# jarek1992/raytracer_project

Measured on AMD Instinct MI355X. Metric: Msamples/sec (rays·bounces), higher is better.
Workload: dtype f64

## Files before the change

### include/zr_capi.h

```cpp
#ifndef ZR_CAPI_H
#define ZR_CAPI_H

#include <stddef.h>
#include <stdint.h>

#ifdef __cplusplus
extern "C" {
#endif

#define ZR_ABI_VERSION 3

enum {
    ZR_OK = 0,
    ZR_E_INVALID = -1,
    ZR_E_DEVICE = -2,
    ZR_E_STATE = -3,
    ZR_E_CANCELLED = -4,
    ZR_E_NOMEM = -5
};

enum {
    ZR_PRIM_SPHERE = 0,
    ZR_PRIM_TRIANGLE = 1,
    ZR_PRIM_CUBE = 2,
// ... 358 lines not shown
    uint32_t leaf;
    uint32_t kind;
    uint32_t count;
    uint32_t first;
    uint32_t subtree;
    uint32_t src[4];
} zr_tree_box;
int zr_scene_tree_boxes(const zr_scene*, zr_tree_box* out, size_t cap);

#define ZR_PATH_RECORD 17
int zr_trace_paths(zr_ctx*, const zr_scene*, const zr_camera*, uint64_t seed, const int32_t* requests, int n, int max_segments, double* out);

int zr_get_counters(zr_ctx*, zr_counters*);
uint64_t zr_last_presolved_pixels(zr_ctx*);
int zr_last_round_loop(zr_ctx*, int* drain_round, int* sub_pools);
int zr_get_kernel_times(zr_ctx*, float* ms, int cap);

#define ZR_COMM_ID_BYTES 128
typedef struct zr_comm zr_comm;
int zr_comm_unique_id(unsigned char id[ZR_COMM_ID_BYTES]);
zr_comm* zr_comm_create(zr_ctx*, int nranks, int rank, const unsigned char id[ZR_COMM_ID_BYTES]);
int zr_comm_reduce_frame(zr_comm*, void* d_frame, size_t n_doubles, int root, void* hip_stream);
int zr_comm_gather_frame(zr_comm*, void* d_frame, int W, int H, const zr_region* region, int root, void* hip_stream);
void zr_comm_destroy(zr_comm*);

int zr_trace(zr_ctx*, const zr_scene*, const double* rays6, size_t n, double tmin, double tmax,
             uint64_t seed, uint64_t pixel, uint32_t bounce, zr_hit* out);

typedef struct zr_scatter_out {
    double attenuation[3], origin[3], direction[3];
// ... 17 lines not shown
```

### raytracer_project_amd/capi.py

```python
import ctypes as C
import os

import numpy as np

_HERE = os.path.dirname(os.path.abspath(__file__))
LIB_PATH = os.environ.get("ZR_LIB") or os.path.join(_HERE, "csrc", "libzr_hip.so")
SCENES_LIB_PATH = os.path.join(_HERE, "csrc", "libzr_scenes.so")

ZR_OK, ZR_E_INVALID, ZR_E_DEVICE, ZR_E_STATE, ZR_E_CANCELLED, ZR_E_NOMEM = 0, -1, -2, -3, -4, -5
NO_TEXTURE = 0xFFFFFFFF


class XformOp(C.Structure):
    _fields_ = [("kind", C.c_uint32), ("mat", C.c_uint32), ("a", C.c_double * 3)]


class Object(C.Structure):
    _fields_ = [("type", C.c_uint32), ("index", C.c_uint32), ("chain_first", C.c_uint32), ("chain_count", C.c_uint32)]


class Medium(C.Structure):
    _fields_ = [("boundary_type", C.c_uint32), ("boundary_index", C.c_uint32), ("chain_first", C.c_uint32),
                ("chain_count", C.c_uint32), ("mat", C.c_uint32), ("pad_", C.c_uint32), ("neg_inv_density", C.c_double)]

# ... 191 lines not shown
_lib = None
_scenes = None

CAPI_SYMBOLS = [
    "zr_abi_version", "zr_last_error", "zr_create", "zr_destroy", "zr_scene_create", "zr_scene_destroy",
    "zr_scene_set_spheres", "zr_scene_set_triangles", "zr_scene_set_triangle_uvs", "zr_scene_set_cubes", "zr_scene_set_media",
    "zr_scene_set_xform_ops", "zr_scene_set_objects", "zr_scene_set_groups", "zr_scene_set_materials", "zr_scene_set_textures",
    "zr_scene_set_all", "zr_scene_set_all_borrowed", "zr_scene_commit", "zr_scene_update_xform_ops", "zr_scene_update_spheres", "zr_scene_refit", "zr_scene_stats", "zr_scene_kernels", "zr_scene_traversal_stack", "zr_scene_builder", "zr_render", "zr_render_device",
    "zr_accum_create", "zr_accum_destroy", "zr_accum_reset", "zr_render_accumulate", "zr_accum_resolve", "zr_accum_resolve_device", "zr_accum_state",
    "zr_render_adaptive", "zr_accum_error", "zr_accum_sample_counts", "zr_accum_lane_sums",
    "zr_render_aov", "zr_render_passes", "zr_trace_paths", "zr_post_process", "zr_analyze_frame", "zr_denoise", "zr_sharpen_frame",
    "zr_accum_variance", "zr_denoise_guided", "zr_accum_denoise",
    "zr_accum_halves", "zr_denoise_nlm", "zr_accum_denoise_nlm",
    "zr_render_gbuffer", "zr_temporal_create", "zr_temporal_destroy", "zr_temporal_reset", "zr_temporal_state", "zr_temporal_accumulate", "zr_accum_temporal",
    "zr_temporal_view",
    "zr_render_bvh_debug", "zr_trace_bvh_debug", "zr_scene_tree_boxes", "zr_get_counters", "zr_last_presolved_pixels", "zr_last_round_loop",
    "zr_get_kernel_times", "zr_trace", "zr_kat_scatter", "zr_kat_shade_lean", "zr_kat_texture", "zr_kat_background", "zr_kat_camera_rays", "zr_comm_unique_id", "zr_comm_create", "zr_comm_reduce_frame", "zr_comm_gather_frame", "zr_comm_destroy",
]


def load():
    global _lib
    if _lib is not None:
        return _lib
    if not os.path.exists(LIB_PATH):
        raise OSError(f"{LIB_PATH} not built: run `python -c 'import __graft_entry__ as g; g.build()'` "
                      "(hipcc --offload-arch=gfx950); there is no CPU fallback")
    lib = C.CDLL(LIB_PATH, mode=C.RTLD_GLOBAL)
    vp, u64, i32 = C.c_void_p, C.c_uint64, C.c_int
    lib.zr_abi_version.restype = i32
    lib.zr_last_error.restype = C.c_char_p
# ... 54 lines not shown
        lib.zr_temporal_reset.argtypes = [vp]
        lib.zr_temporal_state.argtypes = [vp, C.POINTER(C.c_int64 * 4)]
        lib.zr_temporal_accumulate.argtypes = [vp, C.POINTER(TemporalParams), vp, C.POINTER(Camera), u64, vp, vp, vp, vp, vp]
        lib.zr_accum_temporal.argtypes = [vp, vp, C.POINTER(TemporalParams), vp, C.POINTER(Camera), u64, vp, vp, vp]
        lib.zr_temporal_view.argtypes = [C.POINTER(Camera), C.POINTER(C.c_double * 16)]
    lib.zr_render_bvh_debug.argtypes = [vp, vp, C.POINTER(Camera), C.POINTER(Env), u64, C.POINTER(Region), C.POINTER(BvhDebugParams), vp, vp, vp]
    lib.zr_trace_bvh_debug.argtypes = [vp, vp, C.POINTER(BvhDebugParams), vp, C.c_size_t, C.c_double, u64, u64, C.c_uint32, vp]
    lib.zr_scene_tree_boxes.argtypes = [vp, vp, C.c_size_t]
    lib.zr_trace_paths.argtypes = [vp, vp, C.POINTER(Camera), u64, vp, i32, i32, vp]
    lib.zr_render_passes.argtypes = [vp, vp, C.POINTER(Camera), C.POINTER(Env), u64, C.POINTER(Region), vp, vp, vp]
    lib.zr_get_counters.argtypes = [vp, C.POINTER(Counters)]
    if hasattr(lib, "zr_last_presolved_pixels"):
        lib.zr_last_presolved_pixels.argtypes = [vp]; lib.zr_last_presolved_pixels.restype = u64
    if hasattr(lib, "zr_last_round_loop"):
        lib.zr_last_round_loop.argtypes = [vp, C.POINTER(C.c_int), C.POINTER(C.c_int)]
    lib.zr_get_kernel_times.argtypes = [vp, C.POINTER(C.c_float), i32]
    lib.zr_trace.argtypes = [vp, vp, vp, C.c_size_t, C.c_double, C.c_double, u64, u64, C.c_uint32, vp]
    lib.zr_kat_scatter.argtypes = [vp, vp, vp, vp, vp, vp, C.c_size_t, vp]
    if hasattr(lib, "zr_kat_shade_lean"):
        lib.zr_kat_shade_lean.argtypes = [vp, vp, vp, vp, vp, C.c_size_t, vp, vp]
    lib.zr_kat_texture.argtypes = [vp, vp, C.c_uint32, vp, C.c_size_t, vp]
    lib.zr_kat_background.argtypes = [vp, vp, C.POINTER(Env), vp, C.c_size_t, vp]
    lib.zr_kat_camera_rays.argtypes = [vp, C.POINTER(Camera), u64, vp, C.c_size_t, vp]
    lib.zr_comm_unique_id.argtypes = [vp]
    lib.zr_comm_create.restype = vp; lib.zr_comm_create.argtypes = [vp, i32, i32, vp]
    lib.zr_comm_reduce_frame.argtypes = [vp, vp, C.c_size_t, i32, vp]
    lib.zr_comm_gather_frame.argtypes = [vp, vp, i32, i32, C.POINTER(Region), i32, vp]
    lib.zr_comm_destroy.argtypes = [vp]
    _lib = lib
    return lib
# ... 258 lines not shown
        return out

    def counters(self):
        c = Counters()
        _check(self.lib.zr_get_counters(self._c, C.byref(c)))
        return c

    def presolved_pixels(self):
        return int(self.lib.zr_last_presolved_pixels(self._c))

    def round_loop(self):
        d, k = C.c_int(0), C.c_int(0)
        _check(self.lib.zr_last_round_loop(self._c, C.byref(d), C.byref(k)))
        return d.value, k.value

    def kernel_times_ms(self, cap=256):
        buf = (C.c_float * cap)()
        n = self.lib.zr_get_kernel_times(self._c, buf, cap)
        if n < 0:
            _check(n)
        return [buf[i] for i in range(min(n, cap))]


class Accumulator:

    def __init__(self, ctx, width, height, region=None):
        self.ctx = ctx
        self.lib = ctx.lib
        self.width, self.height = int(width), int(height)
        self._a = self.lib.zr_accum_create(ctx._c, self.width, self.height, C.byref(region) if region is not None else None)
# ... 317 lines not shown
```

### raytracer_project_amd/csrc/zr_host_internal.h

```cpp
#pragma once
#include <hip/hip_runtime_api.h>

#include "zr_build.h"
#include "zr_scene_input.h"
#include "zr_launch.h"

#define HIP_OK(expr)                                                                                         \
    do {                                                                                                     \
        hipError_t e_ = (expr);                                                                              \
        if (e_ != hipSuccess) return fail(ZR_E_DEVICE, "%s failed: %s", #expr, hipGetErrorString(e_));       \
    } while (0)

namespace zr_host {

const double kPi = 3.14159265358979323846;

struct H3 { double x, y, z; };
inline H3 h3(const double* p) { return H3{p[0], p[1], p[2]}; }
inline H3 operator+(H3 a, H3 b) { return H3{a.x + b.x, a.y + b.y, a.z + b.z}; }
inline H3 operator-(H3 a, H3 b) { return H3{a.x - b.x, a.y - b.y, a.z - b.z}; }
inline H3 operator-(H3 a) { return H3{-a.x, -a.y, -a.z}; }
inline H3 operator*(double t, H3 v) { return H3{t * v.x, t * v.y, t * v.z}; }
inline H3 operator*(H3 v, double t) { return t * v; }
inline H3 operator/(H3 v, double t) { return (1 / t) * v; }
// ... 55 lines not shown
    DevBuf<uint32_t> d_kend;
    DevBuf<unsigned char> d_cls;
    DevBuf<unsigned long long> d_cpart;
    DevBuf<unsigned int> d_ctl;
    DevBuf<unsigned char> d_st_overflow;
    uint32_t st_ovf_levels = 0;
    int st_blocks = 0;
    int fused_blocks = 0;
    uint32_t st_slots = 0;
    int st_pools = -1;
    hipEvent_t st_event = nullptr;
    unsigned int* h_active = nullptr;
    unsigned int* h_polls = nullptr;
    hipEvent_t poll_events[zr::POLL_RING * ST_MAX_POOLS] = {};
    int last_drain_round = 0, last_sub_pools = 0;
    std::vector<int32_t> pix_key;
    uint64_t last_rounds = 0;
    int last_path = 0;
    double last_extend_ms = 0, last_shade_ms = 0;
    struct Pending { hipEvent_t a, b; uint64_t render_id; int kind; };
    std::vector<hipEvent_t> pool;
    std::vector<Pending> pending;
    std::vector<float> log;
    int log_kind = 1;
    uint64_t render_id = 0;
    double last_render_ms = 0;
    hipStream_t last_stream = nullptr;
    bool last_counted = false;
    std::mutex trash_m;
    std::thread trash;
// ... 58 lines not shown
```

### raytracer_project_amd/csrc/zr_launch.h

```cpp
#pragma once
#include <hip/hip_runtime.h>
#include <stdint.h>
#include "../../include/zr_capi.h"
#include "zr_round_polls.h"

#define ZR_BLOCK 256

namespace zr {

struct DScene;
struct DCamera;
struct DEnv;

enum { CTR_SAMPLES = 0, CTR_SEGMENTS = 1, CTR_NODES = 2, CTR_SPHERES = 3, CTR_TRIANGLES = 4, CTR_CUBES = 5, CTR_MEDIA = 6, CTR_HITS = 7, CTR_DRAWS = 8,
       CTR_NODE_EXECS = 9, CTR_NODE_LANES = 10, CTR_LEAF_EXECS = 11, CTR_LEAF_LANES = 12,
       CTR_SHADE_EXECS = 13, CTR_SHADE_LANES = 14,
       CTR_ESCAPED = 15,
       CTR_WORDS = 16,
       CTR_HIST = 16, CTR_HIST_WORDS = 24,
       CTR_BLOCK = 48 };
enum { CTR_PROF_EXECS = 1, CTR_PROF_LANES = 2,
       CTR_PROF_WAVE_TICKS = 13,
       CTR_PROF_WAVES = 14 };

// ... 38 lines not shown
};
struct StreamPool {
    void* slots; uint32_t P; void* drain; uint32_t drain_slots, unit_chunk;
};
struct StreamContext {
    unsigned int* ctl; void* overflow; uint32_t ovf_levels; int extend_blocks; unsigned long long* gctr;
    hipStream_t* streams; int n_pools;
    hipEvent_t event; unsigned int* h_active;
    unsigned int* h_polls = nullptr; hipEvent_t* poll_events = nullptr;
};
struct StreamSplit { int mode; void* kend; void* cls; unsigned long long* cpart; };
struct StreamHooks {
    StreamTimer* timer; volatile const uint8_t* keep_going ; StreamProgress* progress;
    int* done_out;
    int* drain_out = nullptr;
};
struct StreamJob { StreamFrame frame; StreamPool pool; StreamContext ctx; StreamSplit split; StreamHooks hooks; };
hipError_t stream_render(const DScene& sc, const StreamJob& job, int leaf_level);
#define ZR_FUSED_OBJECTS 16
struct FusedObjs {
    uint32_t n, pad_;
    uint32_t kind[ZR_FUSED_OBJECTS];
    uint32_t index[ZR_FUSED_OBJECTS];
    double rec[ZR_FUSED_OBJECTS][16];
};
int fused_blocks();
hipError_t fused_render_frame(const DScene& sc, const StreamFrame& frame, const StreamContext& ctx, int blocks, int level, const FusedObjs& objs, const StreamHooks& hooks);
constexpr size_t ACCUM_DOUBLES_PER_PIXEL = 192;
hipError_t launch_accumulate(const double* samples, uint32_t n_pix, uint32_t n, uint32_t sample0, bool flip, double* partial, hipStream_t stream);
hipError_t launch_accum_resolve(const double* partial, const uint32_t* pixels, uint32_t n_pix, int W, int done, int asc_lanes, double* out, hipStream_t stream);
// ... 59 lines not shown
```

### raytracer_project_amd/csrc/zr_render.cpp

```cpp
#include "zr_frame.h"

namespace zr_host {
namespace {

size_t batch_tiles(bool interactive) { return (size_t)std::max(1, (int)env_double("ZR_BATCH_TILES", interactive ? 256 : (double)(1 << 30))); }

void make_camera(const zr_camera& c, zr::DCamera& d) {
    int W = c.image_width < 1 ? 1 : c.image_width, H = c.image_height < 1 ? 1 : c.image_height;
    double aspect = double(W) / H;
    H3 center = h3(c.lookfrom), lookat = h3(c.lookat), vup = h3(c.vup);
    double theta = c.vfov * kPi / 180.0;
    double h = std::tan(theta / 2);
    double vh = 2 * h * c.focus_dist;
    double vw = vh * aspect;
    H3 w = unit(center - lookat);
    H3 u = unit(cross(vup, w));
    H3 v = cross(w, u);
    H3 vu = vw * u;
    H3 vv = vh * -v;
    H3 du = vu / W;
    H3 dv = vv / H;
    H3 ul = center - (c.focus_dist * w) - vu / 2 - vv / 2;
    H3 p00 = ul + 0.5 * (du + dv);
    double rad = c.focus_dist * std::tan((c.defocus_angle / 2) * kPi / 180.0);
// ... 342 lines not shown
        for (int y = r.ya; y < r.yb; y++) for (int x = r.xa; x < r.xb; x++) pix.push_back((uint32_t)x | ((uint32_t)y << 16));
    }
    return pix;
}

bool list_runs_reversed() { return env_double("ZR_STREAM_BOTTOM_UP", 1) != 0; }

int render_stream(zr_ctx* c, const zr_scene* s, const FrameJob& job, int mode) {
    int rc = ZR_OK;
    if (!job.d_list && (rc = upload_pixel_list(c, job.plan))) return rc;
    const uint32_t* pixels = job.d_list ? job.d_list : c->d_pixels.p;
    uint32_t n_pix = job.d_list ? job.n_list : (uint32_t)c->d_pixels.n;
    const uint32_t spp = (uint32_t)job.dc.spp;
    if (c->pending.size() > 65536) { int rr = resolve_times(c); if (rr) return rr; }
    c->render_id++; c->last_stream = job.stream; c->last_counted = job.count; c->last_rounds = 0; c->last_drain_round = 0; c->last_sub_pools = 0;
    HIP_OK(hipMemsetAsync(c->d_ctr.p, 0, zr::CTR_BLOCK * sizeof(unsigned long long), job.stream));
    if (n_pix == 0) return ZR_OK;
    uint64_t units = (uint64_t)n_pix * spp;
    size_t samples_n = (size_t)units * 3;
    if (c->d_partial.n < samples_n) {
        HIP_OK(hipStreamSynchronize(job.stream));
        if (c->d_partial.alloc(samples_n) != ZR_OK) return fail(ZR_E_NOMEM, "no device memory for the per-sample radiance buffer (%zu bytes)", samples_n * sizeof(double));
    }
    hipStream_t streams[ST_MAX_POOLS];
    streams[0] = job.stream;
    for (int k = 1; k < ST_MAX_POOLS; k++) streams[k] = c->sub[k];
    const bool fused = mode == 0 && s->fused_ok && s->leaf_level <= 2 && s->leaf_objects > 0 && (double)s->leaf_objects <= env_double("ZR_FUSED_MAX", ZR_FUSED_OBJECTS) &&
                       env_double("ZR_FUSED", 1) != 0;
    if (mode == 0 && !fused && job.d_out && !job.d_list && !job.count && s->ds.shade_escape && env_double("ZR_SKY_PREPASS", 1) != 0) {
        uint32_t n_walk = n_pix;
// ... 10 lines not shown
    if (fused) {
        if (polled) HIP_OK(hipMemsetAsync(c->d_partial.p, 0, samples_n * sizeof(double), job.stream));
        return render_fused(c, s, sj);
    }
    c->last_path = 2;
    if ((rc = ensure_stack_slabs(c, s))) return rc;
    sj.ctx.overflow = c->d_st_overflow.p; sj.ctx.ovf_levels = c->st_ovf_levels;
    const bool lean_pair = s->leaf_level == 0 && s->ds.shade_lean != 0 && mode == 0;
    if ((rc = size_slot_pool(c, units, spp, lean_pair, job.stream, sj.pool))) return rc;
    if (polled) HIP_OK(hipMemsetAsync(c->d_partial.p, 0, samples_n * sizeof(double), job.stream));
    sj.split.mode = mode;
    if (mode != 0 && (rc = split_buffers(c, units, mode, job.stream, sj.split))) return rc;
    const bool sharded = job.plan.tiles.size() < (size_t)job.plan.tiles_x * job.plan.tiles_y;
    sj.ctx.n_pools = c->st_pools > 0 ? c->st_pools : ((sharded || lean_pair) ? 2 : 1);
    HostTimer timer(c);
    int rounds = 0, drain[2] = {0, 0};
    sj.hooks.timer = &timer; sj.hooks.done_out = &rounds; sj.hooks.drain_out = drain;
    hipError_t e = zr::stream_render(s->ds, sj, s->leaf_level);
    if (e != hipSuccess) return fail(ZR_E_DEVICE, "streaming pipeline failed: %s", hipGetErrorString(e));
    c->last_rounds = (uint64_t)(rounds < 0 ? -rounds : rounds); c->last_drain_round = drain[0]; c->last_sub_pools = drain[1];
    HIP_OK(hipStreamSynchronize(job.stream));
    if (rounds < 0) return fail(ZR_E_CANCELLED, "render cancelled after %d rounds", -rounds);
    return ZR_OK;
}

void camera_frame(const zr_camera& cam, zr::DCamera& dc) { make_camera(cam, dc); }

int trace_device(zr_ctx* c, const zr_scene* s, const double* d_rays, size_t n, double tmin, double tmax, uint64_t seed, uint64_t pixel, uint32_t bounce,
                 zr_hit* d_hits) {
    const char* eng = std::getenv("ZR_TRACE_ENGINE");
    const bool can_extend = c->variant == 2 && s->quad_ok && tmin == 0.001 && tmax == HUGE_VAL && n < (1u << 30);
    if (eng && std::strcmp(eng, "extend") == 0 && !can_extend)
        return fail(ZR_E_INVALID, "ZR_TRACE_ENGINE=extend needs ZR_KERNEL=2, tmin = 0.001, tmax = inf and a scene within the 4-wide tree's limits");
    if (can_extend && !(eng && std::strcmp(eng, "pairs") == 0)) {
        DevBuf<unsigned char> pool;
// ... 205 lines not shown
            std::fprintf(stderr, "[zr] %-5s iterations by ready lanes (1-8 ... 57-64):", names[ph]);
            for (int b = 0; b < 8; b++) std::fprintf(stderr, " %5.1f%%", tot ? 100.0 * (double)hh[ph * 8 + b] / (double)tot : 0.0);
            std::fprintf(stderr, "   of %llu\n", tot);
        }
    }
    return ZR_OK;
}

int zr_last_round_loop(zr_ctx* c, int* drain_round, int* sub_pools) {
    if (!c) return fail(ZR_E_INVALID, "null argument");
    if (drain_round) *drain_round = c->last_drain_round;
    if (sub_pools) *sub_pools = c->last_sub_pools;
    return ZR_OK;
}

uint64_t zr_last_presolved_pixels(zr_ctx* c) {
    return c && c->presolved_render == c->render_id ? c->presolved : 0;
}

int zr_get_kernel_times(zr_ctx* c, float* ms, int cap) {
    if (!c) return fail(ZR_E_INVALID, "null argument");
    HIP_OK(hipSetDevice(c->device));
    int rc = resolve_times(c);
    if (rc) return rc;
    int total = (int)c->log.size();
    int n = std::min(total, std::max(cap, 0));
    for (int k = 0; k < n; k++) ms[k] = c->log[c->log.size() - n + k];
    c->log.clear();
    return total;
}
// ... 81 lines not shown
```

### raytracer_project_amd/csrc/zr_stream.hip

```cpp
#include "zr_device.h"
#include "zr_launch.h"

namespace zr {

#ifndef ST_EXT_WAVES
#define ST_EXT_WAVES 4
#endif
#ifndef ST_CHUNK
#define ST_CHUNK 256
#endif
#ifndef ST_SHADE_WAVES
#define ST_SHADE_WAVES 4
#endif
#ifndef ST_EXT_WAVES_LEAN
#define ST_EXT_WAVES_LEAN 6
#endif
#ifndef ST_EXT_WAVES_MID
#define ST_EXT_WAVES_MID 4
#endif
#ifndef ST_FETCH_MIN
#define ST_FETCH_MIN 16
#endif
#define ST_SHARDS 64
#ifndef ST_LDS_STACK
// ... 56 lines not shown
}


__host__ __device__ inline unsigned long long st_unit_of(uint32_t G, uint32_t unit_base, uint32_t shard, unsigned long long k) {
    if (G == 0) return (unsigned long long)unit_base + k * ST_SHARDS + shard;
    const uint32_t k32 = (uint32_t)k, q = k32 / G, r = k32 - q * G;
    const uint32_t pos = (shard & 7u) * (ST_SHARDS / 8u) + (shard >> 3);
    return ((unsigned long long)q * ST_SHARDS + pos) * G + r;
}
__host__ __device__ inline unsigned long long st_first_unit(uint32_t G, uint32_t g) {
    if (G == 0) return g;
    const uint32_t c = g >> 8;
    return st_unit_of(G, 0, c % ST_SHARDS, (unsigned long long)(c / ST_SHARDS) * 256u + (g & 255u));
}

__device__ inline void begin_sample(const StreamBuf& B, const DCamera& cam, uint64_t seed, const SlotAt& S, uint32_t unit, uint32_t& c_samp) {
    const uint32_t pix_i = unit / B.spp, sample = unit - pix_i * B.spp + B.sample0;
    const uint32_t pk = B.pixels[pix_i];
    const int px = (int)(pk & 0xFFFFu), py = (int)(pk >> 16);
    Rng g; g.key = zr_stream_key(seed, (uint64_t)py * (uint64_t)cam.W + (uint64_t)px, (uint64_t)sample); g.k = 0; g.bounce = 0;
    Ray r = camera_ray(cam, px, py, g);
    S.st3(SF_RAY, r.o); S.st3(SF_RAY + 3, r.d);
    S.st(SF_KEY, __longlong_as_double((long long)g.key));
    uint2 ma; ma.x = (uint32_t)g.k; ma.y = F_FIRST | F_ACTIVE;
    uint2 mb; mb.x = unit; mb.y = 0;
    S.st2(SF_MA, ma); S.st2(SF_MB, mb);
    c_samp++;
}

template <bool COUNT>
__global__ __launch_bounds__(256) void stream_init(StreamBuf B, DCamera cam, uint64_t seed, unsigned long long* __restrict__ gctr) {
    const uint32_t slot = blockIdx.x * 256 + threadIdx.x;
    if (slot >= B.P) return;
    uint32_t c_samp = 0;
    const unsigned long long u0 = st_first_unit(B.unit_chunk, B.unit0 + slot);
    const SlotAt S = slot_at(B, blockIdx.x, threadIdx.x);
    if (u0 < (unsigned long long)B.n_units) begin_sample(B, cam, seed, S, (uint32_t)u0, c_samp);
    else { uint2 z; z.x = 0; z.y = 0; S.st2(SF_MA, z); }
    if (COUNT && c_samp) atomicAdd(&gctr[CTR_SAMPLES], (unsigned long long)c_samp);
}

enum { X_IDLE = 0, X_NODE = 1, X_LEAF = 2 };
// ... 268 lines not shown
    if (COUNT) {
        atomicAdd(&gctr[CTR_SEGMENTS], (unsigned long long)c_seg);
        atomicAdd(&gctr[CTR_NODES], (unsigned long long)c_nodes);
        atomicAdd(&gctr[CTR_SPHERES], (unsigned long long)c_sph);
        atomicAdd(&gctr[CTR_TRIANGLES], (unsigned long long)c_tri);
        atomicAdd(&gctr[CTR_CUBES], (unsigned long long)c_cube);
        atomicAdd(&gctr[CTR_MEDIA], (unsigned long long)c_med);
        atomicAdd(&gctr[CTR_HITS], (unsigned long long)c_hits);
        if (lane == 0) for (int k = 0; k < 2; k++) { atomicAdd(&gctr[CTR_NODE_EXECS + 2 * k], s_exec[k]); atomicAdd(&gctr[CTR_NODE_LANES + 2 * k], s_lanes[k]); }
    }
}

#ifndef ST_SHADE_WAVES_LEAN
#define ST_SHADE_WAVES_LEAN 6
#endif
template <bool COUNT, int MODE, bool LEAN = false, bool UV = false>
__global__ __launch_bounds__(256, LEAN ? ST_SHADE_WAVES_LEAN : ST_SHADE_WAVES) void stream_shade(DScene sc, DCamera cam, DEnv env, uint64_t seed, StreamBuf B,
                                                    unsigned long long* __restrict__ gctr) {
    const uint32_t slot0 = blockIdx.x * 256 + threadIdx.x;
    if (slot0 < ST_SHARDS) B.ctl[CTL_SHARD0 + CTL_STRIDE * slot0 + CTL_SH_CHUNK] = 0;
    __shared__ unsigned long long s_cnt[4];
    if (MODE != 0 && threadIdx.x < 4) s_cnt[threadIdx.x] = 0;
    __shared__ unsigned int wave_cls[4][8];
    __shared__ uint4 x_mk[256];
    __shared__ unsigned char x_src[256];
    uint32_t src;
    uint2 m, ki;
    {
        uint2 m0; m0.x = 0; m0.y = 0;
        uint2 k0; k0.x = 0xFFFFFFFFu; k0.y = 0;
        if (slot0 < B.P) { const SlotAt S0 = slot_at(B, blockIdx.x, threadIdx.x); m0 = S0.ld2(SF_MA); k0 = S0.ld2(SF_HIT_KI); }
        uint32_t cls = 7;
        if (m0.y & F_ACTIVE) {
            if (k0.x == 0xFFFFFFFFu) cls = 6;
            else {
                cls = 0;
                if (sc.mat_kinds & (sc.mat_kinds - 1u)) {
                    const uint32_t mat = object_material(sc, k0.x, k0.y);
                    cls = mat < sc.n_mats ? sc.mats[mat].kind : 5u;
                    if (cls > 5u) cls = 5u;
                }
            }
        }
// ... 7 lines not shown
            if (cls == c) my_rank = (unsigned int)__popcll(bm & below);
        }
        __syncthreads();
        unsigned int base = 0;
        for (uint32_t c = 0; c < 8; c++)
            for (int k = 0; k < 4; k++)
                if (c < cls || (c == cls && k < w)) base += wave_cls[k][c];
        uint4 mk4; mk4.x = m0.x; mk4.y = m0.y; mk4.z = k0.x; mk4.w = k0.y;
        x_mk[base + my_rank] = mk4;
        x_src[base + my_rank] = (unsigned char)threadIdx.x;
        __syncthreads();
        mk4 = x_mk[threadIdx.x];
        src = x_src[threadIdx.x];
        m.x = mk4.x; m.y = mk4.y; ki.x = mk4.z; ki.y = mk4.w;
    }
    const SlotAt S = slot_at(B, blockIdx.x, src);
    bool active_after = false, want_unit = false;
    uint32_t c_samp = 0, c_seg2 = 0, c_hit2 = 0, c_esc = 0, c_esc_nodes = 0, c_seen = 0; unsigned long long c_draws = 0;
    {
        if (m.y & F_ACTIVE) {
            const uint32_t NONE = 0xFFFFFFFFu;
            const bool first = (m.y & F_FIRST) != 0;
            if (COUNT && LEAN && MODE == 0) c_seen++;
            Ray ray; ray.o = S.ld3(SF_RAY); ray.d = S.ld3(SF_RAY + 3);
            Rng g; g.key = (uint64_t)__double_as_longlong(S.ld(SF_KEY)); g.k = m.x; g.bounce = (m.y & 0xFFu) + 1u;
            const uint2 mb_now = S.ld2(SF_MB);
            const double t_hit = S.ld(SF_HIT_T);
            V3 beta_now = mk(1, 1, 1);
            if (!first && !(m.y & F_BONE)) beta_now = S.ld3(SF_BETA);
            V3 att0_now = mk(0, 0, 0);
            if (!first && ki.x == NONE) att0_now = S.ld3(SF_ATT0);
            int b_inner = (int)((m.y >> 8) & 0xFFu);
            const int depth_inner = cam.max_depth - 1;
            V3 L_now = mk(0, 0, 0);
            bool have_L_now = false;
            auto load_L = [&]() { return have_L_now ? L_now : ((m.y & F_LZERO) ? mk(0, 0, 0) : S.ld3(SF_L)); };
            auto load_beta = [&]() { return beta_now; };
            uint32_t keep_lzero = m.y & F_LZERO;
            if (COUNT && MODE != 0 && !(MODE == 2 && first)) { c_seg2++; if (ki.x != 0xFFFFFFFFu) c_hit2++; }
            bool ended = false;
            V3 contrib = mk(0, 0, 0);
            V3 add_now = mk(0, 0, 0);
// ... 86 lines not shown
                }
                if (!ended && esc) {
                    escaped = true; miss_first = false;
                    ray = nr;
                    if (COUNT) { c_esc++; c_esc_nodes += esc_nodes; }
                } else if (!ended) {
                    S.st3(SF_RAY, nr.o); S.st3(SF_RAY + 3, nr.d);
                    if (has_add) S.st3(SF_SUM, add_now);
                    m.x = (uint32_t)g.k;
                    m.y = (g.bounce & 0xFFu) | ((uint32_t)b_inner << 8) | F_ACTIVE | (first ? (has_add ? F_L0 : 0u) : (m.y & F_L0)) |
                          (first ? (F_LZERO | F_BONE) : keep_lzero);
                    S.st2(SF_MA, m);
                    active_after = true;
                }
            }
            if (ESC && (ki.x == NONE || escaped)) ZR_MISS_STAGE()
#undef ZR_MISS_STAGE
            if (ended) {
                V3 rad = contrib;
                if (has_add) rad = add_now + rad;
                else if (MODE != 2 && !first && (m.y & F_L0)) rad = S.ld3(SF_SUM) + rad;
                const uint2 mb = mb_now;
                const uint32_t unit = mb.x;
                if (MODE != 2 || !no_output) {
                    double* pp = B.samples + (size_t)unit * 3;
                    pp[0] = rad.x; pp[1] = rad.y; pp[2] = rad.z;
                }
                if (MODE == 1) { uint2 ke; ke.x = (uint32_t)g.k; ke.y = g.bounce; B.kend[unit] = ke; }
                if (MODE == 2 && !no_output) B.cls[unit] = (unsigned char)mb.y;
                if (COUNT) {
                    if (MODE != 2) c_draws += g.k;
                    else if (!(first && ki.x == NONE)) c_draws += g.k - B.kend[unit].x;
                }
                want_unit = true;
            }
        }
    }
    {
        const unsigned long long wm = __ballot(want_unit);
        if (wm != 0ull) {
            const uint32_t shard = blockIdx.x % ST_SHARDS;
            const int wl = threadIdx.x & 63;
            uint32_t k0 = 0;
            if (wl == (int)__builtin_ctzll(wm)) k0 = atomicAdd(&B.uctl[CTL_STRIDE * shard + CTL_SH_UNITS], (unsigned int)__popcll(wm));
            k0 = __shfl(k0, (int)__builtin_ctzll(wm), 64);
            if (want_unit) {
                const unsigned long long k = (unsigned long long)k0 + (unsigned long long)__popcll(wm & ((1ull << wl) - 1ull));
                const unsigned long long u = st_unit_of(B.unit_chunk, B.unit_base, shard, (unsigned long long)B.shard_k0 + k);
                if (u < (unsigned long long)B.n_units) { begin_sample(B, cam, seed, S, (uint32_t)u, c_samp); active_after = true; }
                else { uint2 z; z.x = 0; z.y = 0; S.st2(SF_MA, z); }
            }
        }
    }
    const unsigned long long am = __ballot(active_after);
    if ((threadIdx.x & 63) == 0 && am != 0ull) atomicAdd(&B.ctl[CTL_SHARD0 + CTL_STRIDE * (blockIdx.x % ST_SHARDS) + CTL_SH_ACTIVE], (unsigned int)__popcll(am));
    if (COUNT && MODE == 0) {
        if (c_samp) atomicAdd(&gctr[CTR_SAMPLES], (unsigned long long)c_samp);
        if (c_draws) atomicAdd(&gctr[CTR_DRAWS], c_draws);
        if (c_seen) atomicAdd(&gctr[CTR_SHADE_LANES], (unsigned long long)c_seen);
        if (c_esc) {
            atomicAdd(&gctr[CTR_SEGMENTS], (unsigned long long)c_esc); atomicAdd(&gctr[CTR_ESCAPED], (unsigned long long)c_esc);
            atomicAdd(&gctr[CTR_NODES], (unsigned long long)c_esc_nodes);
        }
    }
    if (MODE != 0) {
        if (c_samp) atomicAdd(&s_cnt[0], (unsigned long long)c_samp);
        if (c_seg2) atomicAdd(&s_cnt[1], (unsigned long long)c_seg2);
        if (c_hit2) atomicAdd(&s_cnt[2], (unsigned long long)c_hit2);
        if (c_draws) atomicAdd(&s_cnt[3], c_draws);
        __syncthreads();
// ... 425 lines not shown
    const size_t cpart_blocks = (size_t)P / 256 + ST_MAX_POOLS + 1;
    if (job.split.cpart && (e = hipMemsetAsync(job.split.cpart, 0, cpart_blocks * 4 * sizeof(unsigned long long), stream)) != hipSuccess) return e;
    auto init = [&](const StreamBuf& B, hipStream_t st) {
        if (H.timer) H.timer->begin(st, 0);
        if (F.count) hipLaunchKernelGGL(stream_init<true>, dim3((B.P + 255) / 256), dim3(256), 0, st, B, cam, F.seed, X.gctr);
        else hipLaunchKernelGGL(stream_init<false>, dim3((B.P + 255) / 256), dim3(256), 0, st, B, cam, F.seed, X.gctr);
        if (H.timer) H.timer->end(st, 0);
    };
    auto extend = [&](const StreamBuf& B, void* o, hipStream_t st) {
        const int eb = (int)((B.P + 63) / 64 < (uint32_t)X.extend_blocks ? (B.P + 63) / 64 : (uint32_t)X.extend_blocks);
        if (H.timer) H.timer->begin(st, 1);
        if (F.count) launch_extend<true>(sc, B, o, X.ovf_levels, eb, X.gctr, leaf_level, st); else launch_extend<false>(sc, B, o, X.ovf_levels, eb, X.gctr, leaf_level, st);
        if (H.timer) H.timer->end(st, 1);
    };
    static const unsigned shade_pad = std::getenv("ZR_SHADE_LDS_PAD") ? (unsigned)std::atoi(std::getenv("ZR_SHADE_LDS_PAD")) : 0u;
    auto shade = [&](const StreamBuf& B, hipStream_t st) {
        if (H.timer) H.timer->begin(st, 2);
        const dim3 sg((B.P + 255) / 256), sb(256);
        if (sc.shade_lean && mode == 0) {
            if (F.count) hipLaunchKernelGGL((stream_shade<true, 0, true>), sg, sb, 0, st, sc, cam, env, F.seed, B, X.gctr);
            else hipLaunchKernelGGL((stream_shade<false, 0, true>), sg, sb, shade_pad, st, sc, cam, env, F.seed, B, X.gctr);
        }
        else if (sc.tri_uv_at) {
            if (mode == 1) hipLaunchKernelGGL((stream_shade<true, 1, false, true>), sg, sb, 0, st, sc, cam, env, F.seed, B, X.gctr);
            else if (mode == 2) hipLaunchKernelGGL((stream_shade<true, 2, false, true>), sg, sb, 0, st, sc, cam, env, F.seed, B, X.gctr);
            else if (F.count) hipLaunchKernelGGL((stream_shade<true, 0, false, true>), sg, sb, 0, st, sc, cam, env, F.seed, B, X.gctr);
            else hipLaunchKernelGGL((stream_shade<false, 0, false, true>), sg, sb, shade_pad, st, sc, cam, env, F.seed, B, X.gctr);
        }
        else if (shade_pad && mode == 0 && !F.count) hipLaunchKernelGGL((stream_shade<false, 0>), sg, sb, shade_pad, st, sc, cam, env, F.seed, B, X.gctr);
        else if (mode == 1) hipLaunchKernelGGL((stream_shade<true, 1>), sg, sb, 0, st, sc, cam, env, F.seed, B, X.gctr);
        else if (mode == 2) hipLaunchKernelGGL((stream_shade<true, 2>), sg, sb, 0, st, sc, cam, env, F.seed, B, X.gctr);
        else if (F.count) hipLaunchKernelGGL((stream_shade<true, 0>), sg, sb, 0, st, sc, cam, env, F.seed, B, X.gctr);
        else hipLaunchKernelGGL((stream_shade<false, 0>), sg, sb, 0, st, sc, cam, env, F.seed, B, X.gctr);
        if (H.timer) H.timer->end(st, 2);
// ... 38 lines not shown
    int rounds = start_rounds, drain_round = 0;
    int check_every = H.progress ? 2 : 8;
    bool cancelled = false, drained = false, capped = false;
    static const bool trace_polls = std::getenv("ZR_STREAM_POLL_TRACE") != nullptr;
    if (!cadenced) for (;;) {
        while (rp.may_enqueue() && e == hipSuccess) enqueue_round(true);
        if (e != hipSuccess) break;
        const int s = rp.slot(rp.oldest());
        PollResult p;
        for (int k = 0; k < rp.pools[s] && e == hipSuccess; k++) {
            e = hipEventSynchronize(poll_event(s, k));
            p.add(poll_words(s, k));
        }
        if (e != hipSuccess) break;
        const RoundPolls::Action a = rp.take(p, P, job.pool.drain_slots, job.pool.drain != nullptr);
        if (trace_polls) std::fprintf(stderr, "[zr] poll of round %d (%d queued behind it): active %llu, units left %d, drain condition %d%s\n", rp.polled, rp.in_flight(),
                                      p.active, (int)p.units_left, (int)drain_condition(p, P, job.pool.drain_slots), a.drain ? " -> compaction" : "");
        if (a.finished) break;
        if (a.drain) {
            const int newest = rp.slot(rp.enqueued);
            for (int k = 1; k < K && e == hipSuccess; k++) e = hipStreamWaitEvent(stream, poll_event(newest, k), 0);
            if (e != hipSuccess) break;
            compact_to_drain(a.drain_P);
            drained = true; drain_round = rp.enqueued;
        }
        if (rp.enqueued > (1 << 22)) { e = hipErrorLaunchFailure; break; }
    }
    if (!cadenced && e == hipSuccess) {
        const int newest = rp.slot(rp.enqueued);
        for (int k = 1; k < K && e == hipSuccess; k++) e = hipStreamWaitEvent(stream, poll_event(newest, k), 0);
// ... 32 lines not shown
                    const unsigned long long c0 = (q * ST_SHARDS + pos) * unit_chunk, len = q < full ? unit_chunk : part;
                    if (c0 < n_units) started += c0 + len <= n_units ? len : n_units - c0;
                }
            }
            if (started > n_units) started = n_units;
            const double frac = started > active ? (double)(started - active) / (double)n_units : 0.0;
            bool reduced = false;
            if (mode == 0 && F.out && H.progress->wants_frame()) {
                hipLaunchKernelGGL(stream_reduce, dim3((n_pix + 3) / 4), dim3(256), 0, stream, Q[0], cam, F.out);
                if ((e = hipStreamSynchronize(stream)) != hipSuccess) break;
                reduced = true;
            }
            H.progress->report(frac, reduced);
        }
        if (active == 0) break;
        if (!drained && job.pool.drain && active * 16ull <= (unsigned long long)P && active <= (unsigned long long)job.pool.drain_slots) {
            bool units_left = false;
            for (int sh = 0; sh < ST_SHARDS && !units_left; sh++)
                if (st_unit_of(unit_chunk, P, (uint32_t)sh, (unsigned long long)(unit_chunk ? P / ST_SHARDS : 0u) + h_units[CTL_STRIDE * sh + CTL_SH_UNITS]) < (unsigned long long)n_units) units_left = true;
            if (!units_left) {
                compact_to_drain(drain_pool_slots(active));
                if (trace_polls) std::fprintf(stderr, "[zr] compaction behind round %d\n", rp.enqueued);
                if ((e = hipStreamSynchronize(stream)) != hipSuccess) break;
                drained = true; drain_round = rp.enqueued;
            }
        }
        check_every = active > P / 2 ? 8 : (active > P / 16 ? 4 : 2);
        if (H.progress && check_every > 2) check_every = 2;
        if (H.keep_going && *H.keep_going == 0) { cancelled = true; break; }
        if (rounds > (1 << 22)) { e = hipErrorLaunchFailure; break; }
    }
    if (e != hipSuccess) return e;
    if (capped) return hipErrorLaunchFailure;
    if (rp.emptied != 0) {
        rounds = start_rounds + rp.emptied;
        if (H.timer) H.timer->drop_from(rp.log_keep());
    }
    const StreamBuf& A = Q[0];
    if (H.timer) H.timer->begin(stream, 3);
    if (job.split.cpart) hipLaunchKernelGGL(stream_sum_counters, dim3(1), dim3(256), 0, stream, job.split.cpart, cpart_blocks, X.gctr);
    if (mode == 2) hipLaunchKernelGGL(stream_reduce_split, dim3((n_pix + 3) / 4), dim3(256), 0, stream, A, cam, F.out, F.out2);
    else if (F.out) hipLaunchKernelGGL(stream_reduce, dim3((n_pix + 3) / 4), dim3(256), 0, stream, A, cam, F.out);
    if (H.timer) H.timer->end(stream, 3);
    if (H.done_out) *H.done_out = cancelled ? -rounds : rounds;
    if (H.drain_out) { H.drain_out[0] = drain_round; H.drain_out[1] = K0; }
    return hipGetLastError();
}

int fused_blocks() {
    int dev = 0, cus = 256, per_cu = 2;
    if (hipGetDevice(&dev) == hipSuccess) { hipDeviceProp_t p; if (hipGetDeviceProperties(&p, dev) == hipSuccess) cus = p.multiProcessorCount; }
    if (hipOccupancyMaxActiveBlocksPerMultiprocessor(&per_cu, fused_render<2, false>, 256, 0) != hipSuccess || per_cu < 1) per_cu = 2;
    return cus * per_cu;
}
hipError_t fused_render_frame(const DScene& sc, const StreamFrame& F, const StreamContext& X, int blocks, int level, const FusedObjs& fo, const StreamHooks& H) {
    const DCamera& cam = *F.cam; const DEnv& env = *F.env;
    hipStream_t stream = X.streams[0];
    const uint32_t n_units = F.n_pix * F.spp;
    const size_t W = stream_ctl_words();
    hipError_t e;
// ... 73 lines not shown
```

Measured before the change: 6981.

## Add in-place unsorted lean shade path with early unit reservation

Adds a SORT=false variant of the lean shade kernel. It skips the per-block LDS material/hit sort, launches 64-thread blocks that each map to a quarter of a 256-slot block, and loads ray state once up front. It is used only when the scene has a single material kind and sample units remain. Wavefronts also reserve the next sample unit with a ballot and atomic before the miss stage, so the pixel lookup can overlap the shading tail. The aim is to remove sort overhead and sync where sorting gives nothing, at the cost of another kernel instantiation and extra host bookkeeping to track whether units are left.

```diff
diff --git a/include/zr_capi.h b/include/zr_capi.h
--- a/include/zr_capi.h
+++ b/include/zr_capi.h
@@ -396,6 +396,7 @@
 int zr_get_counters(zr_ctx*, zr_counters*);
 uint64_t zr_last_presolved_pixels(zr_ctx*);
 int zr_last_round_loop(zr_ctx*, int* drain_round, int* sub_pools);
+int zr_last_shade_builds(zr_ctx*, int* in_place, int* sorted);
 int zr_get_kernel_times(zr_ctx*, float* ms, int cap);
 
 #define ZR_COMM_ID_BYTES 128
diff --git a/raytracer_project_amd/capi.py b/raytracer_project_amd/capi.py
--- a/raytracer_project_amd/capi.py
+++ b/raytracer_project_amd/capi.py
@@ -229,7 +229,7 @@
     "zr_accum_halves", "zr_denoise_nlm", "zr_accum_denoise_nlm",
     "zr_render_gbuffer", "zr_temporal_create", "zr_temporal_destroy", "zr_temporal_reset", "zr_temporal_state", "zr_temporal_accumulate", "zr_accum_temporal",
     "zr_temporal_view",
-    "zr_render_bvh_debug", "zr_trace_bvh_debug", "zr_scene_tree_boxes", "zr_get_counters", "zr_last_presolved_pixels", "zr_last_round_loop",
+    "zr_render_bvh_debug", "zr_trace_bvh_debug", "zr_scene_tree_boxes", "zr_get_counters", "zr_last_presolved_pixels", "zr_last_round_loop", "zr_last_shade_builds",
     "zr_get_kernel_times", "zr_trace", "zr_kat_scatter", "zr_kat_shade_lean", "zr_kat_texture", "zr_kat_background", "zr_kat_camera_rays", "zr_comm_unique_id", "zr_comm_create", "zr_comm_reduce_frame", "zr_comm_gather_frame", "zr_comm_destroy",
 ]
 
@@ -314,6 +314,8 @@
         lib.zr_last_presolved_pixels.argtypes = [vp]; lib.zr_last_presolved_pixels.restype = u64
     if hasattr(lib, "zr_last_round_loop"):
         lib.zr_last_round_loop.argtypes = [vp, C.POINTER(C.c_int), C.POINTER(C.c_int)]
+    if hasattr(lib, "zr_last_shade_builds"):
+        lib.zr_last_shade_builds.argtypes = [vp, C.POINTER(C.c_int), C.POINTER(C.c_int)]
     lib.zr_get_kernel_times.argtypes = [vp, C.POINTER(C.c_float), i32]
     lib.zr_trace.argtypes = [vp, vp, vp, C.c_size_t, C.c_double, C.c_double, u64, u64, C.c_uint32, vp]
     lib.zr_kat_scatter.argtypes = [vp, vp, vp, vp, vp, vp, C.c_size_t, vp]
@@ -602,6 +604,11 @@
         _check(self.lib.zr_last_round_loop(self._c, C.byref(d), C.byref(k)))
         return d.value, k.value
 
+    def shade_builds(self):
+        a, b = C.c_int(0), C.c_int(0)
+        _check(self.lib.zr_last_shade_builds(self._c, C.byref(a), C.byref(b)))
+        return a.value, b.value
+
     def kernel_times_ms(self, cap=256):
         buf = (C.c_float * cap)()
         n = self.lib.zr_get_kernel_times(self._c, buf, cap)
diff --git a/raytracer_project_amd/csrc/zr_host_internal.h b/raytracer_project_amd/csrc/zr_host_internal.h
--- a/raytracer_project_amd/csrc/zr_host_internal.h
+++ b/raytracer_project_amd/csrc/zr_host_internal.h
@@ -93,6 +93,7 @@
     unsigned int* h_polls = nullptr;
     hipEvent_t poll_events[zr::POLL_RING * ST_MAX_POOLS] = {};
     int last_drain_round = 0, last_sub_pools = 0;
+    int last_shade_launches[2] = {0, 0};
     std::vector<int32_t> pix_key;
     uint64_t last_rounds = 0;
     int last_path = 0;
diff --git a/raytracer_project_amd/csrc/zr_launch.h b/raytracer_project_amd/csrc/zr_launch.h
--- a/raytracer_project_amd/csrc/zr_launch.h
+++ b/raytracer_project_amd/csrc/zr_launch.h
@@ -76,6 +76,7 @@
     StreamTimer* timer; volatile const uint8_t* keep_going ; StreamProgress* progress;
     int* done_out;
     int* drain_out = nullptr;
+    int* shade_out = nullptr;
 };
 struct StreamJob { StreamFrame frame; StreamPool pool; StreamContext ctx; StreamSplit split; StreamHooks hooks; };
 hipError_t stream_render(const DScene& sc, const StreamJob& job, int leaf_level);
diff --git a/raytracer_project_amd/csrc/zr_render.cpp b/raytracer_project_amd/csrc/zr_render.cpp
--- a/raytracer_project_amd/csrc/zr_render.cpp
+++ b/raytracer_project_amd/csrc/zr_render.cpp
@@ -380,6 +380,7 @@
     const uint32_t spp = (uint32_t)job.dc.spp;
     if (c->pending.size() > 65536) { int rr = resolve_times(c); if (rr) return rr; }
     c->render_id++; c->last_stream = job.stream; c->last_counted = job.count; c->last_rounds = 0; c->last_drain_round = 0; c->last_sub_pools = 0;
+    c->last_shade_launches[0] = c->last_shade_launches[1] = 0;
     HIP_OK(hipMemsetAsync(c->d_ctr.p, 0, zr::CTR_BLOCK * sizeof(unsigned long long), job.stream));
     if (n_pix == 0) return ZR_OK;
     uint64_t units = (uint64_t)n_pix * spp;
@@ -420,11 +421,12 @@
     const bool sharded = job.plan.tiles.size() < (size_t)job.plan.tiles_x * job.plan.tiles_y;
     sj.ctx.n_pools = c->st_pools > 0 ? c->st_pools : ((sharded || lean_pair) ? 2 : 1);
     HostTimer timer(c);
-    int rounds = 0, drain[2] = {0, 0};
-    sj.hooks.timer = &timer; sj.hooks.done_out = &rounds; sj.hooks.drain_out = drain;
+    int rounds = 0, drain[2] = {0, 0}, shade_launches[2] = {0, 0};
+    sj.hooks.timer = &timer; sj.hooks.done_out = &rounds; sj.hooks.drain_out = drain; sj.hooks.shade_out = shade_launches;
     hipError_t e = zr::stream_render(s->ds, sj, s->leaf_level);
     if (e != hipSuccess) return fail(ZR_E_DEVICE, "streaming pipeline failed: %s", hipGetErrorString(e));
     c->last_rounds = (uint64_t)(rounds < 0 ? -rounds : rounds); c->last_drain_round = drain[0]; c->last_sub_pools = drain[1];
+    c->last_shade_launches[0] = shade_launches[0]; c->last_shade_launches[1] = shade_launches[1];
     HIP_OK(hipStreamSynchronize(job.stream));
     if (rounds < 0) return fail(ZR_E_CANCELLED, "render cancelled after %d rounds", -rounds);
     return ZR_OK;
@@ -660,6 +662,13 @@
     return ZR_OK;
 }
 
+int zr_last_shade_builds(zr_ctx* c, int* in_place, int* sorted) {
+    if (!c) return fail(ZR_E_INVALID, "null argument");
+    if (in_place) *in_place = c->last_shade_launches[0];
+    if (sorted) *sorted = c->last_shade_launches[1];
+    return ZR_OK;
+}
+
 uint64_t zr_last_presolved_pixels(zr_ctx* c) {
     return c && c->presolved_render == c->render_id ? c->presolved : 0;
 }
diff --git a/raytracer_project_amd/csrc/zr_stream.hip b/raytracer_project_amd/csrc/zr_stream.hip
--- a/raytracer_project_amd/csrc/zr_stream.hip
+++ b/raytracer_project_amd/csrc/zr_stream.hip
@@ -1,5 +1,8 @@
 #include "zr_device.h"
 #include "zr_launch.h"
+#ifdef ZR_SHADE_ASSERT
+#include <cassert>
+#endif
 
 namespace zr {
 
@@ -94,9 +97,7 @@
     return st_unit_of(G, 0, c % ST_SHARDS, (unsigned long long)(c / ST_SHARDS) * 256u + (g & 255u));
 }
 
-__device__ inline void begin_sample(const StreamBuf& B, const DCamera& cam, uint64_t seed, const SlotAt& S, uint32_t unit, uint32_t& c_samp) {
-    const uint32_t pix_i = unit / B.spp, sample = unit - pix_i * B.spp + B.sample0;
-    const uint32_t pk = B.pixels[pix_i];
+__device__ __forceinline__ void begin_sample_at(const DCamera& cam, uint64_t seed, const SlotAt& S, uint32_t unit, uint32_t sample, uint32_t pk, uint32_t& c_samp) {
     const int px = (int)(pk & 0xFFFFu), py = (int)(pk >> 16);
     Rng g; g.key = zr_stream_key(seed, (uint64_t)py * (uint64_t)cam.W + (uint64_t)px, (uint64_t)sample); g.k = 0; g.bounce = 0;
     Ray r = camera_ray(cam, px, py, g);
@@ -106,6 +107,15 @@
     uint2 mb; mb.x = unit; mb.y = 0;
     S.st2(SF_MA, ma); S.st2(SF_MB, mb);
     c_samp++;
+}
+__device__ inline void begin_sample(const StreamBuf& B, const DCamera& cam, uint64_t seed, const SlotAt& S, uint32_t unit, uint32_t& c_samp) {
+    const uint32_t pix_i = unit / B.spp, sample = unit - pix_i * B.spp + B.sample0;
+    const uint32_t pk = B.pixels[pix_i];
+    begin_sample_at(cam, seed, S, unit, sample, pk, c_samp);
+}
+__device__ inline void begin_sample(const StreamBuf& B, const DCamera& cam, uint64_t seed, const SlotAt& S, uint32_t unit, uint32_t pk, uint32_t& c_samp) {
+    const uint32_t pix_i = unit / B.spp, sample = unit - pix_i * B.spp + B.sample0;
+    begin_sample_at(cam, seed, S, unit, sample, pk, c_samp);
 }
 
 template <bool COUNT>
@@ -404,10 +414,12 @@
 #ifndef ST_SHADE_WAVES_LEAN
 #define ST_SHADE_WAVES_LEAN 6
 #endif
-template <bool COUNT, int MODE, bool LEAN = false, bool UV = false>
-__global__ __launch_bounds__(256, LEAN ? ST_SHADE_WAVES_LEAN : ST_SHADE_WAVES) void stream_shade(DScene sc, DCamera cam, DEnv env, uint64_t seed, StreamBuf B,
+template <bool COUNT, int MODE, bool LEAN = false, bool UV = false, bool SORT = true>
+__global__ __launch_bounds__(SORT ? 256 : 64, LEAN ? ST_SHADE_WAVES_LEAN : ST_SHADE_WAVES) void stream_shade(DScene sc, DCamera cam, DEnv env, uint64_t seed, StreamBuf B,
                                                     unsigned long long* __restrict__ gctr) {
-    const uint32_t slot0 = blockIdx.x * 256 + threadIdx.x;
+    constexpr bool QUARTER = !SORT;
+    const uint32_t sblock = QUARTER ? blockIdx.x >> 2 : blockIdx.x, sthread = QUARTER ? (blockIdx.x & 3u) * 64u + threadIdx.x : threadIdx.x;
+    const uint32_t slot0 = sblock * 256 + sthread;
     if (slot0 < ST_SHARDS) B.ctl[CTL_SHARD0 + CTL_STRIDE * slot0 + CTL_SH_CHUNK] = 0;
     __shared__ unsigned long long s_cnt[4];
     if (MODE != 0 && threadIdx.x < 4) s_cnt[threadIdx.x] = 0;
@@ -416,7 +428,18 @@
     __shared__ unsigned char x_src[256];
     uint32_t src;
     uint2 m, ki;
-    {
+    Ray ray_in; double key_in, t_in; uint2 mb_in;
+    if constexpr (!SORT) {
+        static_assert(LEAN && MODE == 0, "the in-place build exists for the lean render only");
+        src = sthread;
+        m.x = 0; m.y = 0; ki.x = 0xFFFFFFFFu; ki.y = 0;
+        if (slot0 < B.P) {
+            const SlotAt S0 = slot_at(B, sblock, sthread);
+            m = S0.ld2(SF_MA); ki = S0.ld2(SF_HIT_KI); t_in = S0.ld(SF_HIT_T);
+            ray_in.o = S0.ld3(SF_RAY); ray_in.d = S0.ld3(SF_RAY + 3);
+            key_in = S0.ld(SF_KEY); mb_in = S0.ld2(SF_MB);
+        }
+    } else {
         uint2 m0; m0.x = 0; m0.y = 0;
         uint2 k0; k0.x = 0xFFFFFFFFu; k0.y = 0;
         if (slot0 < B.P) { const SlotAt S0 = slot_at(B, blockIdx.x, threadIdx.x); m0 = S0.ld2(SF_MA); k0 = S0.ld2(SF_HIT_KI); }
@@ -454,18 +477,25 @@
         src = x_src[threadIdx.x];
         m.x = mk4.x; m.y = mk4.y; ki.x = mk4.z; ki.y = mk4.w;
     }
-    const SlotAt S = slot_at(B, blockIdx.x, src);
+    const SlotAt S = slot_at(B, sblock, src);
     bool active_after = false, want_unit = false;
     uint32_t c_samp = 0, c_seg2 = 0, c_hit2 = 0, c_esc = 0, c_esc_nodes = 0, c_seen = 0; unsigned long long c_draws = 0;
+    constexpr uint32_t ST_NO_UNIT = 0xFFFFFFFFu;
+    constexpr bool RESERVE_EARLY = LEAN && MODE == 0 && !SORT;
+    uint32_t next_unit = ST_NO_UNIT, next_pk = 0;
+#ifdef ZR_SHADE_ASSERT
+    bool reserved = false;
+#endif
     {
         if (m.y & F_ACTIVE) {
             const uint32_t NONE = 0xFFFFFFFFu;
             const bool first = (m.y & F_FIRST) != 0;
             if (COUNT && LEAN && MODE == 0) c_seen++;
-            Ray ray; ray.o = S.ld3(SF_RAY); ray.d = S.ld3(SF_RAY + 3);
-            Rng g; g.key = (uint64_t)__double_as_longlong(S.ld(SF_KEY)); g.k = m.x; g.bounce = (m.y & 0xFFu) + 1u;
-            const uint2 mb_now = S.ld2(SF_MB);
-            const double t_hit = S.ld(SF_HIT_T);
+            Ray ray;
+            if constexpr (SORT) { ray.o = S.ld3(SF_RAY); ray.d = S.ld3(SF_RAY + 3); } else ray = ray_in;
+            Rng g; g.key = (uint64_t)__double_as_longlong(SORT ? S.ld(SF_KEY) : key_in); g.k = m.x; g.bounce = (m.y & 0xFFu) + 1u;
+            const uint2 mb_now = SORT ? S.ld2(SF_MB) : mb_in;
+            const double t_hit = SORT ? S.ld(SF_HIT_T) : t_in;
             V3 beta_now = mk(1, 1, 1);
             if (!first && !(m.y & F_BONE)) beta_now = S.ld3(SF_BETA);
             V3 att0_now = mk(0, 0, 0);
@@ -582,6 +612,25 @@
                     active_after = true;
                 }
             }
+            if constexpr (RESERVE_EARLY) {
+                const bool will_end = ended || ki.x == NONE || escaped;
+                const unsigned long long wm = __ballot(will_end);
+                if (wm != 0ull) {
+                    const uint32_t shard = sblock % ST_SHARDS;
+                    const int wl = threadIdx.x & 63, first_lane = (int)__builtin_ctzll(wm);
+                    uint32_t k0 = 0;
+                    if (wl == first_lane) k0 = atomicAdd(&B.uctl[CTL_STRIDE * shard + CTL_SH_UNITS], (unsigned int)__popcll(wm));
+                    k0 = __shfl(k0, first_lane, 64);
+                    if (will_end) {
+                        const unsigned long long k = (unsigned long long)k0 + (unsigned long long)__popcll(wm & ((1ull << wl) - 1ull));
+                        const unsigned long long u = st_unit_of(B.unit_chunk, B.unit_base, shard, (unsigned long long)B.shard_k0 + k);
+                        if (u < (unsigned long long)B.n_units) { next_unit = (uint32_t)u; next_pk = B.pixels[next_unit / B.spp]; }
+                    }
+                }
+#ifdef ZR_SHADE_ASSERT
+                reserved = will_end;
+#endif
+            }
             if (ESC && (ki.x == NONE || escaped)) ZR_MISS_STAGE()
 #undef ZR_MISS_STAGE
             if (ended) {
@@ -604,10 +653,18 @@
             }
         }
     }
-    {
+    if constexpr (RESERVE_EARLY) {
+#ifdef ZR_SHADE_ASSERT
+        assert(want_unit == reserved);
+#endif
+        if (want_unit) {
+            if (next_unit != ST_NO_UNIT) { begin_sample(B, cam, seed, S, next_unit, next_pk, c_samp); active_after = true; }
+            else { uint2 z; z.x = 0; z.y = 0; S.st2(SF_MA, z); }
+        }
+    } else {
         const unsigned long long wm = __ballot(want_unit);
         if (wm != 0ull) {
-            const uint32_t shard = blockIdx.x % ST_SHARDS;
+            const uint32_t shard = sblock % ST_SHARDS;
             const int wl = threadIdx.x & 63;
             uint32_t k0 = 0;
             if (wl == (int)__builtin_ctzll(wm)) k0 = atomicAdd(&B.uctl[CTL_STRIDE * shard + CTL_SH_UNITS], (unsigned int)__popcll(wm));
@@ -621,7 +678,7 @@
         }
     }
     const unsigned long long am = __ballot(active_after);
-    if ((threadIdx.x & 63) == 0 && am != 0ull) atomicAdd(&B.ctl[CTL_SHARD0 + CTL_STRIDE * (blockIdx.x % ST_SHARDS) + CTL_SH_ACTIVE], (unsigned int)__popcll(am));
+    if ((threadIdx.x & 63) == 0 && am != 0ull) atomicAdd(&B.ctl[CTL_SHARD0 + CTL_STRIDE * (sblock % ST_SHARDS) + CTL_SH_ACTIVE], (unsigned int)__popcll(am));
     if (COUNT && MODE == 0) {
         if (c_samp) atomicAdd(&gctr[CTR_SAMPLES], (unsigned long long)c_samp);
         if (c_draws) atomicAdd(&gctr[CTR_DRAWS], c_draws);
@@ -1077,10 +1134,21 @@
         if (H.timer) H.timer->end(st, 1);
     };
     static const unsigned shade_pad = std::getenv("ZR_SHADE_LDS_PAD") ? (unsigned)std::atoi(std::getenv("ZR_SHADE_LDS_PAD")) : 0u;
+    const char* in_place_env = std::getenv("ZR_SHADE_IN_PLACE");
+    const bool in_place_ok = sc.shade_lean && mode == 0 && (sc.mat_kinds & (sc.mat_kinds - 1u)) == 0 && !(in_place_env && std::atoi(in_place_env) == 0);
+    bool units_left = true;
+    int shade_launches[2] = {0, 0};
     auto shade = [&](const StreamBuf& B, hipStream_t st) {
         if (H.timer) H.timer->begin(st, 2);
         const dim3 sg((B.P + 255) / 256), sb(256);
-        if (sc.shade_lean && mode == 0) {
+        const bool in_place = in_place_ok && units_left;
+        shade_launches[in_place ? 0 : 1]++;
+        if (in_place) {
+            const dim3 sg((B.P + 255) / 256 * 4), sb(64);
+            if (F.count) hipLaunchKernelGGL((stream_shade<true, 0, true, false, false>), sg, sb, 0, st, sc, cam, env, F.seed, B, X.gctr);
+            else hipLaunchKernelGGL((stream_shade<false, 0, true, false, false>), sg, sb, shade_pad, st, sc, cam, env, F.seed, B, X.gctr);
+        }
+        else if (sc.shade_lean && mode == 0) {
             if (F.count) hipLaunchKernelGGL((stream_shade<true, 0, true>), sg, sb, 0, st, sc, cam, env, F.seed, B, X.gctr);
             else hipLaunchKernelGGL((stream_shade<false, 0, true>), sg, sb, shade_pad, st, sc, cam, env, F.seed, B, X.gctr);
         }
@@ -1149,6 +1217,7 @@
         }
         if (e != hipSuccess) break;
         const RoundPolls::Action a = rp.take(p, P, job.pool.drain_slots, job.pool.drain != nullptr);
+        units_left = p.units_left;
         if (trace_polls) std::fprintf(stderr, "[zr] poll of round %d (%d queued behind it): active %llu, units left %d, drain condition %d%s\n", rp.polled, rp.in_flight(),
                                       p.active, (int)p.units_left, (int)drain_condition(p, P, job.pool.drain_slots), a.drain ? " -> compaction" : "");
         if (a.finished) break;
@@ -1211,10 +1280,12 @@
             H.progress->report(frac, reduced);
         }
         if (active == 0) break;
-        if (!drained && job.pool.drain && active * 16ull <= (unsigned long long)P && active <= (unsigned long long)job.pool.drain_slots) {
-            bool units_left = false;
+        if (units_left) {
+            units_left = false;
             for (int sh = 0; sh < ST_SHARDS && !units_left; sh++)
                 if (st_unit_of(unit_chunk, P, (uint32_t)sh, (unsigned long long)(unit_chunk ? P / ST_SHARDS : 0u) + h_units[CTL_STRIDE * sh + CTL_SH_UNITS]) < (unsigned long long)n_units) units_left = true;
+        }
+        if (!drained && job.pool.drain && active * 16ull <= (unsigned long long)P && active <= (unsigned long long)job.pool.drain_slots) {
             if (!units_left) {
                 compact_to_drain(drain_pool_slots(active));
                 if (trace_polls) std::fprintf(stderr, "[zr] compaction behind round %d\n", rp.enqueued);
@@ -1241,6 +1312,7 @@
     if (H.timer) H.timer->end(stream, 3);
     if (H.done_out) *H.done_out = cancelled ? -rounds : rounds;
     if (H.drain_out) { H.drain_out[0] = drain_round; H.drain_out[1] = K0; }
+    if (H.shade_out) { H.shade_out[0] = shade_launches[0]; H.shade_out[1] = shade_launches[1]; }
     return hipGetLastError();
 }
 
```

Result: faster. 7119, median of 6 (+2.0%).
